# intelligent-machine-learning/dlrover

Measured on AMD Instinct MI355X. Metric: checkpoint save+restore sec and goodput % under injected failure, Llama-3-8B FSDP 1/2/4/8 MI355X, higher is better.
Workload: dtype bf16; 1 GPU; model=llama3_8b, params=8030261248, global_batch=2, seq_len=4096, parallelism=fsdp1, ckpt_interval=2, ckpt_scope=full, ckpt_restored_step=1

## Files before the change

dlrover_amd/ops/api.py:

```python

from typing import Optional, Tuple

import torch

_EXT = None
_EXT_ERR: Optional[str] = None


class ExtensionMissingError(RuntimeError):
    pass


def hip_ops():
    global _EXT, _EXT_ERR
    if _EXT is None and _EXT_ERR is None:
        try:
            from dlrover_amd.ops import _hip_ops as ext

            _EXT = ext
        except ImportError as e:
            _EXT_ERR = str(e)
    if _EXT is None:
        raise ExtensionMissingError(
            "dlrover_amd._hip_ops is not built — run "
# ... 208 lines not shown
    max_pos: int, head_dim: int, base: float = 500000.0, device="cpu"
) -> Tuple[torch.Tensor, torch.Tensor]:
    inv_freq = 1.0 / (
        base ** (torch.arange(0, head_dim, 2, dtype=torch.float32) / head_dim)
    )
    t = torch.arange(max_pos, dtype=torch.float32)
    freqs = torch.outer(t, inv_freq)
    return freqs.cos().to(device), freqs.sin().to(device)


class _CausalSoftmax(torch.autograd.Function):
    @staticmethod
    def forward(ctx, scores, scale, q_offset, q_len):
        q_len = q_len or scores.shape[-2]
        if _use_hip(scores):
            probs = scores.contiguous()
            hip_ops().causal_softmax_fwd(probs, q_len, q_offset, scale)
        else:
            probs = causal_softmax_ref(scores, scale, q_offset, q_len)
        ctx.save_for_backward(probs)
        ctx.scale = scale
        return probs

    @staticmethod
    def backward(ctx, dprobs):
        (probs,) = ctx.saved_tensors
        if _use_hip(probs):
            ds = dprobs.contiguous().clone()
            hip_ops().causal_softmax_bwd(ds, probs, ctx.scale)
            return ds, None, None, None
        pf, df = probs.float(), dprobs.float()
        dot = (pf * df).sum(-1, keepdim=True)
        return (pf * (df - dot) * ctx.scale).to(probs.dtype), None, None, None


def causal_softmax(
    scores: torch.Tensor, scale: float, q_offset: int = 0, q_len: int = 0
) -> torch.Tensor:
    return _CausalSoftmax.apply(scores, scale, q_offset, q_len)


def flash_attention_ref(
    q: torch.Tensor, k: torch.Tensor, v: torch.Tensor, scale: float
) -> torch.Tensor:
    B, H, S, D = q.shape
    rep = H // k.shape[1]
    kf = k.float().repeat_interleave(rep, 1)
    vf = v.float().repeat_interleave(rep, 1)
    s_ = torch.matmul(q.float(), kf.transpose(-1, -2)) * scale
    mask = torch.triu(torch.ones(S, S, dtype=torch.bool, device=q.device), 1)
    s_ = s_.masked_fill(mask, float("-inf"))
    p = torch.softmax(s_, -1)
    return torch.matmul(p, vf).to(q.dtype)


class _FlashAttention(torch.autograd.Function):
    @staticmethod
    def forward(ctx, q, k, v, scale):
        if _use_hip(q):
            if q.stride(-1) != 1:
                q = q.contiguous()
            if k.stride(-1) != 1:
                k = k.contiguous()
            if v.stride(-1) != 1:
                v = v.contiguous()
            out, lse = hip_ops().flash_attn_fwd(q, k, v, scale)
            ctx.save_for_backward(q, k, v, out, lse)
            ctx.scale = scale
            ctx.use_hip = True
            return out
        ctx.use_hip = False
        q32 = q.detach().clone().requires_grad_(True)
        k32 = k.detach().clone().requires_grad_(True)
        v32 = v.detach().clone().requires_grad_(True)
        with torch.enable_grad():
            out = flash_attention_ref(q32, k32, v32, scale)
        ctx.saved_ref = (q32, k32, v32, out)
        return out.detach()

    @staticmethod
    def backward(ctx, dout):
        if ctx.use_hip:
            q, k, v, out, lse = ctx.saved_tensors
            dq, dk, dv = hip_ops().flash_attn_bwd(
                q, k, v, out, dout.contiguous(), lse, ctx.scale
            )
            return dq, dk, dv, None
        q32, k32, v32, out = ctx.saved_ref
        torch.autograd.backward(out, dout)
        return q32.grad, k32.grad, v32.grad, None


def flash_attention(
    q: torch.Tensor, k: torch.Tensor, v: torch.Tensor, scale: float
) -> torch.Tensor:
    return _FlashAttention.apply(q, k, v, scale)


class _CrossEntropy(torch.autograd.Function):
    @staticmethod
    def forward(ctx, logits, targets, ignore_index):
        n_valid = int((targets != ignore_index).sum())
        grad_scale = 1.0 / max(n_valid, 1)
        if _use_hip(logits):
            work = logits.contiguous()
            losses = hip_ops().cross_entropy_fwd_bwd(
                work, targets.int(), ignore_index, grad_scale, True
            )
            ctx.save_for_backward(work)
            ctx.use_hip = True
        else:
            lf = logits.float()
            losses = torch.nn.functional.cross_entropy(
                lf.view(-1, lf.shape[-1]),
                targets.view(-1).long(),
                ignore_index=ignore_index,
                reduction="none",
            )
            dl = torch.softmax(lf, dim=-1)
            t = targets.view(-1)
            valid = t != ignore_index
            onehot = torch.zeros_like(dl.view(-1, dl.shape[-1]))
            onehot[valid, t[valid].long()] = 1.0
            dl = (dl.view(-1, dl.shape[-1]) - onehot) * grad_scale
            dl[~valid] = 0
            ctx.save_for_backward(dl.to(logits.dtype).view_as(logits))
            ctx.use_hip = False
        ctx.n_valid = n_valid
        return losses.sum() * grad_scale

    @staticmethod
    def backward(ctx, dloss):
        (dlogits,) = ctx.saved_tensors
        return dlogits * dloss, None, None


def cross_entropy_loss(
    logits: torch.Tensor, targets: torch.Tensor, ignore_index: int = -100
) -> torch.Tensor:
    return _CrossEntropy.apply(logits, targets, ignore_index)




def ce_shard_stats(
    logits_shard: torch.Tensor,
    targets: torch.Tensor,
    vocab_start: int,
    ignore_index: int = -100,
) -> torch.Tensor:
    vs = logits_shard.shape[-1]
    if _use_hip(logits_shard):
        return hip_ops().ce_shard_stats(
            logits_shard.view(-1, vs), targets.reshape(-1).int(), vocab_start,
            ignore_index,
        )
    x = logits_shard.detach().reshape(-1, vs).float()
    t = targets.reshape(-1).long()
    m = x.amax(-1)
    s = torch.exp(x - m[:, None]).sum(-1)
    local = t - vocab_start
    owns = (t != ignore_index) & (local >= 0) & (local < vs)
    picked = x.gather(1, torch.where(owns, local, 0)[:, None]).squeeze(1)
    return torch.stack([m, s, torch.where(owns, picked, 0.0)], dim=1)


def ce_shard_finish(
    logits_shard: torch.Tensor,
# ... 231 lines not shown
```

dlrover_amd/ops/csrc/attention_bwd_v3.hip:

```cpp
#include <cstdlib>
#include "kern_common.h"

typedef __attribute__((ext_vector_type(8))) __bf16 bf16x8;
typedef __attribute__((ext_vector_type(16))) float f32x16_t;
typedef __attribute__((ext_vector_type(2))) unsigned int u32x2_t;
typedef __attribute__((ext_vector_type(4))) unsigned int u32x4_t;
typedef __attribute__((ext_vector_type(2))) __bf16 bf16x2;

#define FB_D 128
#define FB_QB 256
#define FB_T 64

__device__ __forceinline__ int swzb(int row, int byte_col) {
  return byte_col ^ ((row & 7) << 4);
}

__device__ __forceinline__ unsigned pk_bf16(float lo, float hi) {
  bf16x2 v = {(__bf16)lo, (__bf16)hi};
  return *reinterpret_cast<unsigned*>(&v);
}

__device__ __forceinline__ bf16x8 trT_frag(const char* lds, int rb, int n,
                                           int lane, int half) {
  const int j = (lane & 15) >> 2;
  const int dq = n * 8 + ((lane & 16) >> 2) + (lane & 3);
  const int r0 = rb + half * 8 + j;
  const int r1 = r0 + 4;
  const unsigned base = (unsigned)(uintptr_t)lds;
  const unsigned a0 = base + r0 * 256 + ((dq * 8) ^ ((r0 & 7) << 4));
  const unsigned a1 = base + r1 * 256 + ((dq * 8) ^ ((r1 & 7) << 4));
  u32x2_t w0, w1;
  asm volatile(
      "ds_read_b64_tr_b16 %0, %2\n\t"
      "ds_read_b64_tr_b16 %1, %3\n\t"
      "s_waitcnt lgkmcnt(0)"
      : "=v"(w0), "=v"(w1)
      : "v"(a0), "v"(a1));
  u32x4_t frag = u32x4_t{w0.x, w0.y, w1.x, w1.y};
  return *reinterpret_cast<bf16x8*>(&frag);
}

__device__ __forceinline__ void pairswap_frags(const float v16[16], int half,
                                               bf16x8 out[2]) {
#pragma unroll
  for (int ks2 = 0; ks2 < 2; ++ks2) {
    const int r0 = ks2 * 8;
    unsigned w0 = pk_bf16(v16[r0 + 0], v16[r0 + 1]);
    unsigned w1 = pk_bf16(v16[r0 + 2], v16[r0 + 3]);
    unsigned w2 = pk_bf16(v16[r0 + 4], v16[r0 + 5]);
    unsigned w3 = pk_bf16(v16[r0 + 6], v16[r0 + 7]);
    u32x2_t s0 = __builtin_amdgcn_permlane32_swap(w0, w2, false, false);
    u32x2_t s1 = __builtin_amdgcn_permlane32_swap(w1, w3, false, false);
    u32x4_t frag = u32x4_t{s0.x, s1.x, s0.y, s1.y};
    out[ks2] = *reinterpret_cast<bf16x8*>(&frag);
  }
  (void)half;
}


__global__ __launch_bounds__(512) void fa_bwd_dq_v3_kernel(
    const short* __restrict__ q, const short* __restrict__ k,
    const short* __restrict__ v, const short* __restrict__ dout,
    const float* __restrict__ lse, const float* __restrict__ dvec,
    short* __restrict__ dq, int B, int H, int HKV, int S, float scale,
    long long qs_b, long long qs_h, long long qs_s,
    long long ks_b, long long ks_h, long long ks_s,
    long long vs_b, long long vs_h, long long vs_s,
    long long ds_b, long long ds_h, long long ds_s) {
  __shared__ char k_lds[2][FB_T * FB_D * 2];
  __shared__ char v_lds[2][FB_T * FB_D * 2];

  const int tid = threadIdx.x;
  const int wave = tid >> 6;
  const int lane = tid & 63;
  const int half = lane >> 5;
  const int qcol = lane & 31;

  const int qt = blockIdx.x;
  const int h = blockIdx.y;
  const int b = blockIdx.z;
  const int g = h / (H / HKV);

  const short* q_blk = q + (long long)b * qs_b + (long long)h * qs_h +
                       (long long)(qt * FB_QB) * qs_s;
  const short* do_blk = dout + (long long)b * ds_b + (long long)h * ds_h +
                        (long long)(qt * FB_QB) * ds_s;
  const short* k_head = k + (long long)b * ks_b + (long long)g * ks_h;
  const short* v_head = v + (long long)b * vs_b + (long long)g * vs_h;

  const int q_row_w = wave * 32 + qcol;
  const int q_glob = qt * FB_QB + q_row_w;

  bf16x8 bq[8], bdo[8];
#pragma unroll
  for (int ks = 0; ks < 8; ++ks) {
    bq[ks] = *reinterpret_cast<const bf16x8*>(
        q_blk + (long long)q_row_w * qs_s + ks * 16 + half * 8);
    bdo[ks] = *reinterpret_cast<const bf16x8*>(
        do_blk + (long long)q_row_w * ds_s + ks * 16 + half * 8);
  }
  const long long lrow = ((long long)b * H + h) * S + q_glob;
  const float L = lse[lrow];
  const float Dv = dvec[lrow];

  f32x16_t acc_dq[4];
#pragma unroll
  for (int n = 0; n < 4; ++n)
#pragma unroll
    for (int r = 0; r < 16; ++r) acc_dq[n][r] = 0.f;

  bf16x8 st_k[2], st_v[2];
  const int st_row0 = (tid * 16) / FB_D;
  const int st_col0 = (tid * 16) % FB_D;
  auto issue_loads = [&](int kt) {
    const short* ksrc = k_head + (long long)(kt * FB_T) * ks_s;
    const short* vsrc = v_head + (long long)(kt * FB_T) * vs_s;
#pragma unroll
    for (int c = 0; c < 2; ++c) {
      st_k[c] = *reinterpret_cast<const bf16x8*>(
          ksrc + (long long)st_row0 * ks_s + st_col0 + c * 8);
      st_v[c] = *reinterpret_cast<const bf16x8*>(
          vsrc + (long long)st_row0 * vs_s + st_col0 + c * 8);
    }
  };
  auto write_lds = [&](int buf) {
#pragma unroll
    for (int c = 0; c < 2; ++c) {
      const int col = st_col0 + c * 8;
      *reinterpret_cast<bf16x8*>(k_lds[buf] + st_row0 * 256 +
                                 swzb(st_row0, col * 2)) = st_k[c];
      *reinterpret_cast<bf16x8*>(v_lds[buf] + st_row0 * 256 +
                                 swzb(st_row0, col * 2)) = st_v[c];
    }
  };

  const int n_tiles = (qt + 1) * (FB_QB / FB_T);
  const int wave_q_max = qt * FB_QB + wave * 32 + 31;

  issue_loads(0);
  write_lds(0);
  __syncthreads();

  for (int kt = 0; kt < n_tiles; ++kt) {
    const int cur = kt & 1;
    const char* k_cur = k_lds[cur];
    const char* v_cur = v_lds[cur];
    if (kt + 1 < n_tiles) issue_loads(kt + 1);

    const int kv0 = kt * FB_T;
    if (kv0 <= wave_q_max) {
      bf16x8 bds[4];
#pragma unroll
      for (int n = 0; n < 2; ++n) {
        f32x16_t acc_s;
#pragma unroll
        for (int r = 0; r < 16; ++r) acc_s[r] = 0.f;
#pragma unroll
        for (int ks = 0; ks < 8; ++ks) {
          const int row = n * 32 + qcol;
          bf16x8 ak = *reinterpret_cast<const bf16x8*>(
              k_cur + row * 256 + swzb(row, (ks * 16 + half * 8) * 2));
          acc_s = __builtin_amdgcn_mfma_f32_32x32x16_bf16(ak, bq[ks], acc_s,
                                                          0, 0, 0);
        }
#pragma unroll
        for (int r = 0; r < 16; ++r) {
          const int kv_glob = kv0 + n * 32 + (r & 3) + 8 * (r >> 2) + 4 * half;
          acc_s[r] =
              (kv_glob > q_glob) ? 0.f : __expf(acc_s[r] * scale - L);
        }
        f32x16_t acc_dp;
#pragma unroll
        for (int r = 0; r < 16; ++r) acc_dp[r] = 0.f;
#pragma unroll
        for (int ks = 0; ks < 8; ++ks) {
          const int row = n * 32 + qcol;
          bf16x8 av = *reinterpret_cast<const bf16x8*>(
              v_cur + row * 256 + swzb(row, (ks * 16 + half * 8) * 2));
          acc_dp = __builtin_amdgcn_mfma_f32_32x32x16_bf16(av, bdo[ks],
                                                           acc_dp, 0, 0, 0);
        }
        float dsv[16];
#pragma unroll
        for (int r = 0; r < 16; ++r)
          dsv[r] = acc_s[r] * (acc_dp[r] - Dv) * scale;
        pairswap_frags(dsv, half, &bds[n * 2]);
      }
#pragma unroll
      for (int n = 0; n < 4; ++n) {
#pragma unroll
        for (int ks = 0; ks < 4; ++ks) {
          bf16x8 akT = trT_frag(k_cur, ks * 16, n, lane, half);
          acc_dq[n] = __builtin_amdgcn_mfma_f32_32x32x16_bf16(
              akT, bds[ks], acc_dq[n], 0, 0, 0);
        }
      }
    }

    __syncthreads();
    if (kt + 1 < n_tiles) {
      write_lds(cur ^ 1);
      __syncthreads();
    }
  }

  short* dq_blk = dq + (long long)b * qs_b + (long long)h * qs_h +
                  (long long)(qt * FB_QB) * qs_s;
  char* slab = (char*)k_lds + (wave & 3) * (32 * FB_D * 2);
  for (int round = 0; round < 2; ++round) {
    __syncthreads();
    if ((wave >> 2) == round) {
#pragma unroll
      for (int n = 0; n < 4; ++n) {
#pragma unroll
        for (int r = 0; r < 16; ++r) {
          const int d = n * 32 + (r & 3) + 8 * (r >> 2) + 4 * half;
          *reinterpret_cast<__bf16*>(slab + qcol * 256 + swzb(qcol, d * 2)) =
              (__bf16)acc_dq[n][r];
        }
      }
    }
    __syncthreads();
    if ((wave >> 2) == round) {
#pragma unroll
      for (int pass = 0; pass < 4; ++pass) {
        const int elem0 = (pass * 64 + lane) * 16;
        const int r2 = elem0 / FB_D;
        const int c2 = elem0 % FB_D;
        bf16x8 v0 = *reinterpret_cast<const bf16x8*>(
            slab + r2 * 256 + swzb(r2, c2 * 2));
        bf16x8 v1 = *reinterpret_cast<const bf16x8*>(
            slab + r2 * 256 + swzb(r2, (c2 + 8) * 2));
        short* dst = dq_blk + (long long)(wave * 32 + r2) * qs_s + c2;
        *reinterpret_cast<bf16x8*>(dst) = v0;
        *reinterpret_cast<bf16x8*>(dst + 8) = v1;
      }
    }
  }
}


#define FB_DKV_PROLOGUE()                                                    \
  __shared__ char q_lds[FB_T * FB_D * 2];                                    \
  __shared__ char do_lds[FB_T * FB_D * 2];                                   \
  __shared__ float l_lds[FB_T];                                              \
  __shared__ float d_lds[FB_T];                                              \
  const int tid = threadIdx.x;                                               \
  const int wave = tid >> 6;                                                 \
  const int lane = tid & 63;                                                 \
  const int half = lane >> 5;                                                \
  const int kcol = lane & 31;                                                \
  const int kvb0 = blockIdx.x * FB_QB;                                       \
  const int chunk = blockIdx.y;                                              \
  const int CH = gridDim.y;                                                  \
  const int bg = blockIdx.z;                                                 \
  const int b = bg / HKV;                                                    \
  const int g = bg % HKV;                                                    \
  const int rep = H / HKV;                                                   \
  const int kv_own = kvb0 + wave * 32 + kcol;                                \
  const short* k_head = k + (long long)b * ks_b + (long long)g * ks_h;       \
  bf16x8 bk[8];                                                              \
  _Pragma("unroll") for (int ks = 0; ks < 8; ++ks) bk[ks] =                  \
      *reinterpret_cast<const bf16x8*>(k_head + (long long)kv_own * ks_s +   \
                                       ks * 16 + half * 8);                  \
  const int qt_min = kvb0 / FB_T;                                            \
  const int n_qt = S / FB_T - qt_min;                                        \
  const int n_work = rep * n_qt;                                             \
  const int wave_kv_min = kvb0 + wave * 32;                                  \
  auto stage_qdo = [&](int h, int qt) {                                      \
    const short* qsrc = q + (long long)b * qs_b + (long long)h * qs_h +      \
                        (long long)(qt * FB_T) * qs_s;                       \
    const short* dsrc = dout + (long long)b * ds_b + (long long)h * ds_h +   \
                        (long long)(qt * FB_T) * ds_s;                       \
    _Pragma("unroll") for (int c = 0; c < 2; ++c) {                          \
      const int linear = (tid * 16) + c * 8;                                 \
      const int row = linear / FB_D;                                         \
      const int col = linear % FB_D;                                         \
      *reinterpret_cast<bf16x8*>(q_lds + row * 256 + swzb(row, col * 2)) =   \
          *reinterpret_cast<const bf16x8*>(qsrc + (long long)row * qs_s +    \
                                           col);                             \
      *reinterpret_cast<bf16x8*>(do_lds + row * 256 + swzb(row, col * 2)) =  \
          *reinterpret_cast<const bf16x8*>(dsrc + (long long)row * ds_s +    \
                                           col);                             \
    }                                                                        \
    if (tid < FB_T) {                                                        \
      const long long lrow = ((long long)b * H + h) * S + qt * FB_T + tid;   \
      l_lds[tid] = lse[lrow];                                                \
      d_lds[tid] = dvec[lrow];                                               \
    }                                                                        \
  }

__global__ __launch_bounds__(512) void fa_bwd_dv_v3_kernel(
    const short* __restrict__ q, const short* __restrict__ k,
    const short* __restrict__ v, const short* __restrict__ dout,
    const float* __restrict__ lse, const float* __restrict__ dvec,
    float* __restrict__ dk32, float* __restrict__ dv32, int B, int H,
    int HKV, int S, float scale,
    long long qs_b, long long qs_h, long long qs_s,
    long long ks_b, long long ks_h, long long ks_s,
    long long vs_b, long long vs_h, long long vs_s,
    long long ds_b, long long ds_h, long long ds_s) {
  FB_DKV_PROLOGUE();

  {
    f32x16_t acc_dv[4];
#pragma unroll
    for (int n = 0; n < 4; ++n)
#pragma unroll
      for (int r = 0; r < 16; ++r) acc_dv[n][r] = 0.f;

    for (int w = chunk; w < n_work; w += CH) {
      const int h = g * rep + w / n_qt;
      const int qt = qt_min + w % n_qt;
      __syncthreads();
      stage_qdo(h, qt);
      __syncthreads();
      if (qt * FB_T + FB_T - 1 < wave_kv_min) continue;
#pragma unroll
      for (int st = 0; st < 2; ++st) {
        const int q0 = qt * FB_T + st * 32;
        if (q0 + 31 < wave_kv_min) continue;
        f32x16_t acc_s;
#pragma unroll
        for (int r = 0; r < 16; ++r) acc_s[r] = 0.f;
#pragma unroll
        for (int ks = 0; ks < 8; ++ks) {
          const int row = st * 32 + kcol;
          bf16x8 aq = *reinterpret_cast<const bf16x8*>(
              q_lds + (st * 32 + kcol) * 256 +
              swzb(st * 32 + kcol, (ks * 16 + half * 8) * 2));
          (void)row;
          acc_s = __builtin_amdgcn_mfma_f32_32x32x16_bf16(aq, bk[ks], acc_s,
                                                          0, 0, 0);
        }
        float pv[16];
#pragma unroll
        for (int r = 0; r < 16; ++r) {
          const int qrow = st * 32 + (r & 3) + 8 * (r >> 2) + 4 * half;
          const int q_glob = qt * FB_T + qrow;
          pv[r] = (kv_own > q_glob)
                      ? 0.f
                      : __expf(acc_s[r] * scale - l_lds[qrow]);
        }
        bf16x8 bp[2];
        pairswap_frags(pv, half, bp);
#pragma unroll
        for (int n = 0; n < 4; ++n) {
#pragma unroll
          for (int ks2 = 0; ks2 < 2; ++ks2) {
            bf16x8 adoT =
                trT_frag(do_lds, st * 32 + ks2 * 16, n, lane, half);
            acc_dv[n] = __builtin_amdgcn_mfma_f32_32x32x16_bf16(
                adoT, bp[ks2], acc_dv[n], 0, 0, 0);
          }
        }
      }
    }
    float* dv_base = dv32 + ((long long)bg * S + kv_own) * FB_D;
#pragma unroll
    for (int n = 0; n < 4; ++n)
#pragma unroll
      for (int r = 0; r < 16; ++r) {
        const int d = n * 32 + (r & 3) + 8 * (r >> 2) + 4 * half;
        atomicAdd(dv_base + d, acc_dv[n][r]);
      }
  }

}

__global__ __launch_bounds__(512) void fa_bwd_dk_v3_kernel(
    const short* __restrict__ q, const short* __restrict__ k,
    const short* __restrict__ v, const short* __restrict__ dout,
    const float* __restrict__ lse, const float* __restrict__ dvec,
    float* __restrict__ dk32, float* __restrict__ dv32, int B, int H,
    int HKV, int S, float scale,
    long long qs_b, long long qs_h, long long qs_s,
    long long ks_b, long long ks_h, long long ks_s,
    long long vs_b, long long vs_h, long long vs_s,
    long long ds_b, long long ds_h, long long ds_s) {
  FB_DKV_PROLOGUE();
  const short* v_head = v + (long long)b * vs_b + (long long)g * vs_h;
  bf16x8 bv[8];
#pragma unroll
  for (int ks = 0; ks < 8; ++ks)
    bv[ks] = *reinterpret_cast<const bf16x8*>(
        v_head + (long long)kv_own * vs_s + ks * 16 + half * 8);

  {
    f32x16_t acc_dk[4];
#pragma unroll
    for (int n = 0; n < 4; ++n)
#pragma unroll
      for (int r = 0; r < 16; ++r) acc_dk[n][r] = 0.f;

    for (int w = chunk; w < n_work; w += CH) {
      const int h = g * rep + w / n_qt;
      const int qt = qt_min + w % n_qt;
      __syncthreads();
      stage_qdo(h, qt);
      __syncthreads();
      if (qt * FB_T + FB_T - 1 < wave_kv_min) continue;
#pragma unroll
      for (int st = 0; st < 2; ++st) {
        const int q0 = qt * FB_T + st * 32;
        if (q0 + 31 < wave_kv_min) continue;
        f32x16_t acc_s, acc_dp;
#pragma unroll
        for (int r = 0; r < 16; ++r) acc_s[r] = acc_dp[r] = 0.f;
#pragma unroll
        for (int ks = 0; ks < 8; ++ks) {
          const int row = st * 32 + kcol;
          const int bc = (ks * 16 + half * 8) * 2;
          bf16x8 aq = *reinterpret_cast<const bf16x8*>(
              q_lds + row * 256 + swzb(row, bc));
          acc_s = __builtin_amdgcn_mfma_f32_32x32x16_bf16(aq, bk[ks], acc_s,
                                                          0, 0, 0);
          bf16x8 ado = *reinterpret_cast<const bf16x8*>(
              do_lds + row * 256 + swzb(row, bc));
          acc_dp = __builtin_amdgcn_mfma_f32_32x32x16_bf16(ado, bv[ks],
                                                           acc_dp, 0, 0, 0);
        }
        float dsv[16];
#pragma unroll
        for (int r = 0; r < 16; ++r) {
          const int qrow = st * 32 + (r & 3) + 8 * (r >> 2) + 4 * half;
          const int q_glob = qt * FB_T + qrow;
          const float p = (kv_own > q_glob)
                              ? 0.f
                              : __expf(acc_s[r] * scale - l_lds[qrow]);
          dsv[r] = p * (acc_dp[r] - d_lds[qrow]) * scale;
        }
        bf16x8 bds[2];
        pairswap_frags(dsv, half, bds);
#pragma unroll
        for (int n = 0; n < 4; ++n) {
#pragma unroll
          for (int ks2 = 0; ks2 < 2; ++ks2) {
            bf16x8 aqT = trT_frag(q_lds, st * 32 + ks2 * 16, n, lane, half);
            acc_dk[n] = __builtin_amdgcn_mfma_f32_32x32x16_bf16(
                aqT, bds[ks2], acc_dk[n], 0, 0, 0);
          }
        }
      }
    }
    float* dk_base = dk32 + ((long long)bg * S + kv_own) * FB_D;
#pragma unroll
    for (int n = 0; n < 4; ++n)
#pragma unroll
      for (int r = 0; r < 16; ++r) {
        const int d = n * 32 + (r & 3) + 8 * (r >> 2) + 4 * half;
        atomicAdd(dk_base + d, acc_dk[n][r]);
      }
  }
}

extern "C" void fa_bwd_dkv_v3_launch(const void* q, const void* k,
                                     const void* v, const void* dout,
                                     const void* lse, const void* dvec,
                                     void* dk32, void* dv32, int B, int H,
                                     int HKV, int S, float scale,
                                     const long long* strides,
                                     hipStream_t stream) {
  const int kv_blocks = S / FB_QB;
  int ch = 1;
  while (kv_blocks * ch * B * HKV < 512 && ch < 16) ch <<= 1;
  dim3 grid(kv_blocks, ch, B * HKV);
  hipLaunchKernelGGL(fa_bwd_dv_v3_kernel, grid, dim3(512), 0, stream,
                     (const short*)q, (const short*)k, (const short*)v,
                     (const short*)dout, (const float*)lse,
                     (const float*)dvec, (float*)dk32, (float*)dv32, B, H,
                     HKV, S, scale, strides[0], strides[1], strides[2],
                     strides[3], strides[4], strides[5], strides[6],
                     strides[7], strides[8], strides[9], strides[10],
                     strides[11]);
  hipLaunchKernelGGL(fa_bwd_dk_v3_kernel, grid, dim3(512), 0, stream,
                     (const short*)q, (const short*)k, (const short*)v,
                     (const short*)dout, (const float*)lse,
                     (const float*)dvec, (float*)dk32, (float*)dv32, B, H,
                     HKV, S, scale, strides[0], strides[1], strides[2],
                     strides[3], strides[4], strides[5], strides[6],
                     strides[7], strides[8], strides[9], strides[10],
                     strides[11]);
}

extern "C" void fa_bwd_dq_v3_launch(const void* q, const void* k,
                                    const void* v, const void* dout,
                                    const void* lse, const void* dvec,
                                    void* dq, int B, int H, int HKV, int S,
                                    float scale, const long long* strides,
                                    hipStream_t stream) {
  dim3 grid(S / FB_QB, H, B);
  hipLaunchKernelGGL(fa_bwd_dq_v3_kernel, grid, dim3(512), 0, stream,
                     (const short*)q, (const short*)k, (const short*)v,
                     (const short*)dout, (const float*)lse,
                     (const float*)dvec, (short*)dq, B, H, HKV, S, scale,
                     strides[0], strides[1], strides[2], strides[3],
                     strides[4], strides[5], strides[6], strides[7],
                     strides[8], strides[9], strides[10], strides[11]);
}
```

dlrover_amd/ops/csrc/attention_v3.hip:

```cpp
#include <cstdlib>
#include "kern_common.h"

typedef __attribute__((ext_vector_type(8))) __bf16 bf16x8;
typedef __attribute__((ext_vector_type(4))) float f32x4_t;
typedef __attribute__((ext_vector_type(16))) float f32x16_t;
typedef __attribute__((ext_vector_type(2))) unsigned int u32x2_t;
typedef __attribute__((ext_vector_type(4))) unsigned int u32x4_t;
typedef __attribute__((ext_vector_type(2))) __bf16 bf16x2;

#define FA3_D 128
#define FA3_QB 256
#define FA3_QW 32
#define FA3_KT 64

__device__ __forceinline__ int swz3(int row, int byte_col) {
  return byte_col ^ ((row & 7) << 4);
}

__device__ __forceinline__ unsigned pack_bf16(float lo, float hi) {
  bf16x2 v = {(__bf16)lo, (__bf16)hi};
  return *reinterpret_cast<unsigned*>(&v);
}

__device__ __forceinline__ bf16x8 tr_colT_frag(const char* lds, int rb,
                                               int n, int lane, int half) {
  typedef __attribute__((ext_vector_type(2))) unsigned int u32x2_;
  const int j = (lane & 15) >> 2;
  const int dq = n * 8 + ((lane & 16) >> 2) + (lane & 3);
  const int r0 = rb + half * 8 + j;
  const int r1 = r0 + 4;
  const unsigned base = (unsigned)(uintptr_t)lds;
  const unsigned a0 = base + r0 * 256 + ((dq * 8) ^ ((r0 & 7) << 4));
  const unsigned a1 = base + r1 * 256 + ((dq * 8) ^ ((r1 & 7) << 4));
  u32x2_ w0, w1;
  asm volatile(
      "ds_read_b64_tr_b16 %0, %2\n\t"
      "ds_read_b64_tr_b16 %1, %3\n\t"
      "s_waitcnt lgkmcnt(0)"
      : "=v"(w0), "=v"(w1)
      : "v"(a0), "v"(a1));
  u32x4_t frag = u32x4_t{w0.x, w0.y, w1.x, w1.y};
  return *reinterpret_cast<bf16x8*>(&frag);
}

template <bool TRV>
__global__ __launch_bounds__(512) void flash_attn_fwd_v3_kernel(
    const short* __restrict__ q, const short* __restrict__ k,
    const short* __restrict__ v, short* __restrict__ out,
    float* __restrict__ lse, int B, int H, int HKV, int S, float scale,
    long long qs_b, long long qs_h, long long qs_s,
    long long ks_b, long long ks_h, long long ks_s,
    long long vs_b, long long vs_h, long long vs_s,
    long long os_b, long long os_h, long long os_s) {
  __shared__ char k_lds[2][FA3_KT * FA3_D * 2];
  __shared__ char vt_lds[2][FA3_D * FA3_KT * 2];

  const int tid = threadIdx.x;
  const int wave = tid >> 6;
  const int lane = tid & 63;
  const int half = lane >> 5;
  const int qcol = lane & 31;

  const int qt = blockIdx.x;
  const int h = blockIdx.y;
  const int b = blockIdx.z;
  const int g = h / (H / HKV);

  const short* q_blk = q + (long long)b * qs_b + (long long)h * qs_h +
                       (long long)(qt * FA3_QB) * qs_s;
  const short* k_head = k + (long long)b * ks_b + (long long)g * ks_h;
  const short* v_head = v + (long long)b * vs_b + (long long)g * vs_h;

  const int q_row_w = wave * FA3_QW + qcol;
  bf16x8 bq[8];
#pragma unroll
  for (int ks = 0; ks < 8; ++ks) {
    const short* src =
        q_blk + (long long)q_row_w * qs_s + ks * 16 + half * 8;
    bq[ks] = *reinterpret_cast<const bf16x8*>(src);
  }

  const int q_glob = qt * FA3_QB + q_row_w;
  float m_run = -1e30f, l_run = 0.f;
  f32x16_t acc_o[4];
#pragma unroll
  for (int n = 0; n < 4; ++n)
#pragma unroll
    for (int r = 0; r < 16; ++r) acc_o[n][r] = 0.f;

  bf16x8 st_k[2], st_v[2];
  const int st_row0 = (tid * 16) / FA3_D;
  const int st_col0 = (tid * 16) % FA3_D;

  auto issue_loads = [&](int kt) {
    const short* ksrc = k_head + (long long)(kt * FA3_KT) * ks_s;
    const short* vsrc = v_head + (long long)(kt * FA3_KT) * vs_s;
#pragma unroll
    for (int c = 0; c < 2; ++c) {
      st_k[c] = *reinterpret_cast<const bf16x8*>(
          ksrc + (long long)st_row0 * ks_s + st_col0 + c * 8);
      st_v[c] = *reinterpret_cast<const bf16x8*>(
          vsrc + (long long)st_row0 * vs_s + st_col0 + c * 8);
    }
  };

  auto write_lds = [&](int buf) {
    char* kb = k_lds[buf];
    char* vb = vt_lds[buf];
#pragma unroll
    for (int c = 0; c < 2; ++c) {
      const int col = st_col0 + c * 8;
      *reinterpret_cast<bf16x8*>(kb + st_row0 * 256 + swz3(st_row0, col * 2)) =
          st_k[c];
      if (TRV) {
        *reinterpret_cast<bf16x8*>(vb + st_row0 * 256 +
                                   swz3(st_row0, col * 2)) = st_v[c];
      } else {
#pragma unroll
        for (int i = 0; i < 8; ++i) {
          const int trow = col + i;
          *reinterpret_cast<__bf16*>(vb + trow * 128 +
                                     swz3(trow, st_row0 * 2)) = st_v[c][i];
        }
      }
    }
  };

  const int n_tiles = (qt + 1) * (FA3_QB / FA3_KT);
  const int wave_q_max = qt * FA3_QB + wave * FA3_QW + FA3_QW - 1;

  issue_loads(0);
  write_lds(0);
  __syncthreads();

  for (int kt = 0; kt < n_tiles; ++kt) {
    const int cur = kt & 1;
    const char* k_cur = k_lds[cur];
    const char* vt_cur = vt_lds[cur];
    if (kt + 1 < n_tiles) issue_loads(kt + 1);

    const int kv0 = kt * FA3_KT;
    const bool wave_active = kv0 <= wave_q_max;

    if (wave_active) {
      f32x16_t acc_s[2];
#pragma unroll
      for (int n = 0; n < 2; ++n)
#pragma unroll
        for (int r = 0; r < 16; ++r) acc_s[n][r] = 0.f;
// ... 69 lines not shown
          const int r0 = n * 16 + ks2 * 8;
          unsigned w0 = pack_bf16(p[r0 + 0], p[r0 + 1]);
          unsigned w1 = pack_bf16(p[r0 + 2], p[r0 + 3]);
          unsigned w2 = pack_bf16(p[r0 + 4], p[r0 + 5]);
          unsigned w3 = pack_bf16(p[r0 + 6], p[r0 + 7]);
          u32x2_t s0 = __builtin_amdgcn_permlane32_swap(w0, w2, false, false);
          u32x2_t s1 = __builtin_amdgcn_permlane32_swap(w1, w3, false, false);
          u32x4_t frag = u32x4_t{s0.x, s1.x, s0.y, s1.y};
          bp[n * 2 + ks2] = *reinterpret_cast<bf16x8*>(&frag);
        }
      }

#pragma unroll
      for (int n = 0; n < 4; ++n) {
#pragma unroll
        for (int ks = 0; ks < 4; ++ks) {
          bf16x8 av;
          if (TRV) {
            av = tr_colT_frag(vt_cur, ks * 16, n, lane, half);
          } else {
            const int row = n * 32 + qcol;
            const int byte_col = (ks * 16 + half * 8) * 2;
            av = *reinterpret_cast<const bf16x8*>(
                vt_cur + row * 128 + swz3(row, byte_col));
          }
          acc_o[n] = __builtin_amdgcn_mfma_f32_32x32x16_bf16(av, bp[ks],
                                                             acc_o[n], 0, 0, 0);
        }
      }
    }

    __syncthreads();
    if (kt + 1 < n_tiles) {
      write_lds(cur ^ 1);
      __syncthreads();
    }
  }

  const float inv = l_run > 0.f ? 1.f / l_run : 0.f;
  short* o_blk = out + (long long)b * os_b + (long long)h * os_h +
                 (long long)(qt * FA3_QB) * os_s;
  char* slab = (char*)k_lds + (wave & 3) * (FA3_QW * FA3_D * 2);
  for (int round = 0; round < 2; ++round) {
    __syncthreads();
    if ((wave >> 2) == round) {
#pragma unroll
      for (int n = 0; n < 4; ++n) {
#pragma unroll
        for (int r = 0; r < 16; ++r) {
          const int d = n * 32 + (r & 3) + 8 * (r >> 2) + 4 * half;
          *reinterpret_cast<__bf16*>(slab + qcol * 256 + swz3(qcol, d * 2)) =
              (__bf16)(acc_o[n][r] * inv);
        }
      }
    }
    __syncthreads();
    if ((wave >> 2) == round) {
#pragma unroll
      for (int pass = 0; pass < 4; ++pass) {
        const int elem0 = (pass * 64 + lane) * 16;
        const int r2 = elem0 / FA3_D;
        const int c2 = elem0 % FA3_D;
        bf16x8 v0 = *reinterpret_cast<const bf16x8*>(
            slab + r2 * 256 + swz3(r2, c2 * 2));
        bf16x8 v1 = *reinterpret_cast<const bf16x8*>(
            slab + r2 * 256 + swz3(r2, (c2 + 8) * 2));
        short* dst = o_blk + (long long)(wave * FA3_QW + r2) * os_s + c2;
        *reinterpret_cast<bf16x8*>(dst) = v0;
        *reinterpret_cast<bf16x8*>(dst + 8) = v1;
      }
    }
  }
  if (half == 0 && lse != nullptr) {
    const long long lrow = ((long long)b * H + h) * S + q_glob;
    lse[lrow] = m_run + __logf(fmaxf(l_run, 1e-30f));
  }
}

extern "C" void flash_attn_fwd_v3_launch(const void* q, const void* k,
                                         const void* v, void* out, void* lse,
                                         int B, int H, int HKV, int S,
                                         float scale, const long long* strides,
                                         hipStream_t stream) {
  dim3 grid(S / FA3_QB, H, B);
  static const bool trv = []() {
    const char* e = getenv("DLROVER_FA_TRV");
    return e == nullptr || e[0] != '0';
  }();
  if (trv) {
    hipLaunchKernelGGL((flash_attn_fwd_v3_kernel<true>), grid, dim3(512), 0,
                       stream, (const short*)q, (const short*)k,
                       (const short*)v, (short*)out, (float*)lse, B, H, HKV,
                       S, scale, strides[0], strides[1], strides[2],
                       strides[3], strides[4], strides[5], strides[6],
                       strides[7], strides[8], strides[9], strides[10],
                       strides[11]);
  } else {
    hipLaunchKernelGGL((flash_attn_fwd_v3_kernel<false>), grid, dim3(512), 0,
                       stream, (const short*)q, (const short*)k,
                       (const short*)v, (short*)out, (float*)lse, B, H, HKV,
                       S, scale, strides[0], strides[1], strides[2],
                       strides[3], strides[4], strides[5], strides[6],
                       strides[7], strides[8], strides[9], strides[10],
                       strides[11]);
  }
}
```

dlrover_amd/ops/csrc/bindings.cpp:

```cpp
#include <torch/extension.h>
#include <ATen/cuda/CUDAContext.h>

#include <tuple>
#include <vector>

extern "C" {
void rmsnorm_fwd_launch(const void*, const void*, void*, void*, int, int,
                        float, void*);
void rmsnorm_add_fwd_launch(const void*, const void*, const void*, void*,
                            void*, void*, int, int, float, void*);
void rmsnorm_bwd_launch(const void*, const void*, const void*, const void*,
                        const void*, void*, void*, void*, void*, int, int,
                        int, void*);
void rope_launch(void*, const void*, const void*, const void*, long long,
                 long long, int, int, int, void*);
void rope_oop_launch(const void*, void*, const void*, const void*,
                     const void*, long long, long long, int, int, long long,
                     int, void*);
void swiglu_fwd_launch(const void*, void*, long long, int, void*);
void swiglu_bwd_launch(const void*, const void*, void*, long long, int, void*);
void adamw_launch(void*, const void*, void*, void*, void*, long long, float,
                  float, float, float, float, int, int, float, void*);
void causal_softmax_fwd_launch(void*, long long, int, int, int, float, void*);
void causal_softmax_bwd_launch(void*, const void*, long long, int, float,
// ... 221 lines not shown
  TORCH_CHECK(row_len % 8 == 0, "row_len must be a multiple of 8");
  const long long n_rows = scores.numel() / row_len;
  causal_softmax_fwd_launch(scores.data_ptr(), n_rows, row_len, (int)q_len,
                            (int)q_offset, (float)scale, cur_stream());
}

void causal_softmax_bwd(at::Tensor& dscores, const at::Tensor& probs,
                        double scale) {
  check_bf16(dscores, "dscores");
  check_bf16(probs, "probs");
  const int row_len = (int)dscores.size(-1);
  const long long n_rows = dscores.numel() / row_len;
  causal_softmax_bwd_launch(dscores.data_ptr(), probs.data_ptr(), n_rows,
                            row_len, (float)scale, cur_stream());
}

static void check_attn_view(const at::Tensor& t, const char* name) {
  TORCH_CHECK(t.is_cuda() && t.scalar_type() == at::kBFloat16, name,
              " must be bf16 GPU");
  TORCH_CHECK(t.dim() == 4 && t.stride(3) == 1, name,
              " must be [B,H,S,D] with contiguous D");
}

static void pack_strides(long long* st, const at::Tensor& t, int at) {
  st[at + 0] = (long long)t.stride(0);
  st[at + 1] = (long long)t.stride(1);
  st[at + 2] = (long long)t.stride(2);
}

std::tuple<at::Tensor, at::Tensor> flash_attn_fwd(const at::Tensor& q,
                                                  const at::Tensor& k,
                                                  const at::Tensor& v,
                                                  double scale) {
  check_attn_view(q, "q");
  check_attn_view(k, "k");
  check_attn_view(v, "v");
  const int B = (int)q.size(0), H = (int)q.size(1), S = (int)q.size(2);
  const int D = (int)q.size(3), HKV = (int)k.size(1);
  TORCH_CHECK(D == 128, "flash_attn: head_dim must be 128");
  TORCH_CHECK(S % 64 == 0, "flash_attn: seq len must be a multiple of 64");
  TORCH_CHECK(H % HKV == 0, "flash_attn: H % HKV != 0");
  auto out_bshd = at::empty({B, S, H, D}, q.options());
  auto out = out_bshd.permute({0, 2, 1, 3});
  auto lse = at::empty({B, H, S}, q.options().dtype(at::kFloat));
  long long st[12];
  pack_strides(st, q, 0);
  pack_strides(st, k, 3);
  pack_strides(st, v, 6);
  pack_strides(st, out, 9);
  static const bool use_v2 = []() {
    const char* e = getenv("DLROVER_FA_V2");
    return e != nullptr && e[0] == '1';
  }();
  static const bool v3_enabled = []() {
    const char* e = getenv("DLROVER_FA_V3");
    return e == nullptr || e[0] != '0';
  }();
  if (v3_enabled && !use_v2 && S % 256 == 0) {
    flash_attn_fwd_v3_launch(q.data_ptr(), k.data_ptr(), v.data_ptr(),
                             out_bshd.data_ptr(), lse.data_ptr(), B, H, HKV,
                             S, (float)scale, st, cur_stream());
  } else if (use_v2) {
    flash_attn_fwd_v2_launch(q.data_ptr(), k.data_ptr(), v.data_ptr(),
                             out_bshd.data_ptr(), lse.data_ptr(), B, H, HKV,
                             S, (float)scale, st, cur_stream());
  } else {
    flash_attn_fwd_launch(q.data_ptr(), k.data_ptr(), v.data_ptr(),
                          out_bshd.data_ptr(), lse.data_ptr(), B, H, HKV, S,
                          (float)scale, st, cur_stream());
  }
  return {out, lse};
}

std::tuple<at::Tensor, at::Tensor, at::Tensor> flash_attn_bwd(
    const at::Tensor& q, const at::Tensor& k, const at::Tensor& v,
    const at::Tensor& out, const at::Tensor& dout_in, const at::Tensor& lse,
    double scale) {
  check_attn_view(q, "q");
  check_attn_view(k, "k");
  check_attn_view(v, "v");
  const int B = (int)q.size(0), H = (int)q.size(1), S = (int)q.size(2);
  const int D = (int)q.size(3), HKV = (int)k.size(1);
  at::Tensor dout = dout_in;
  if (dout.strides() != out.strides()) {
    dout = at::empty_like(out.permute({0, 2, 1, 3}).contiguous())
               .view({B, S, H, D});
    dout = dout.permute({0, 2, 1, 3});
    dout.copy_(dout_in);
  }
  TORCH_CHECK(dout.stride(3) == 1, "dout needs contiguous D");
  auto dvec = at::empty({B, H, S}, q.options().dtype(at::kFloat));
  {
    long long ost[3], dstr[3];
    pack_strides(ost, out, 0);
    pack_strides(dstr, dout, 0);
    fa_bwd_pre_launch(dout.data_ptr(), out.data_ptr(), dvec.data_ptr(), B, H,
                      S, ost, dstr, cur_stream());
    long long st[12];
    pack_strides(st, q, 0);
    pack_strides(st, k, 3);
    pack_strides(st, v, 6);
    pack_strides(st, dout, 9);
    auto dq_bshd = at::empty({B, S, H, D}, q.options());
    auto dq = dq_bshd.permute({0, 2, 1, 3});
    {
      long long stq[12];
      pack_strides(stq, dq, 0);
      pack_strides(stq, k, 3);
      pack_strides(stq, v, 6);
      pack_strides(stq, dout, 9);
      at::Tensor quse = q;
      if (q.strides() != dq.strides()) {
        auto q_bshd = at::empty({B, S, H, D}, q.options());
        auto qv = q_bshd.permute({0, 2, 1, 3});
        qv.copy_(q);
        quse = qv;
        pack_strides(stq, quse, 0);
      }
      static const bool bwd_v3 = []() {
        const char* e = getenv("DLROVER_FA_BWD_V3");
        return e == nullptr || e[0] != '0';
      }();
      auto dk32 = at::zeros({B, HKV, S, D}, k.options().dtype(at::kFloat));
      auto dv32 = at::zeros({B, HKV, S, D}, v.options().dtype(at::kFloat));
      if (bwd_v3 && S % 256 == 0) {
        fa_bwd_dq_v3_launch(quse.data_ptr(), k.data_ptr(), v.data_ptr(),
                            dout.data_ptr(), lse.data_ptr(), dvec.data_ptr(),
                            dq_bshd.data_ptr(), B, H, HKV, S, (float)scale,
                            stq, cur_stream());
        fa_bwd_dkv_v3_launch(quse.data_ptr(), k.data_ptr(), v.data_ptr(),
                             dout.data_ptr(), lse.data_ptr(),
                             dvec.data_ptr(), dk32.data_ptr(),
                             dv32.data_ptr(), B, H, HKV, S, (float)scale,
                             stq, cur_stream());
      } else {
        fa_bwd_dq_launch(quse.data_ptr(), k.data_ptr(), v.data_ptr(),
                         dout.data_ptr(), lse.data_ptr(), dvec.data_ptr(),
                         dq_bshd.data_ptr(), B, H, HKV, S, (float)scale, stq,
                         cur_stream());
        fa_bwd_dkv_launch(quse.data_ptr(), k.data_ptr(), v.data_ptr(),
                          dout.data_ptr(), lse.data_ptr(), dvec.data_ptr(),
                          dk32.data_ptr(), dv32.data_ptr(), B, H, HKV, S,
                          (float)scale, stq, cur_stream());
      }
      auto dk = at::empty({B, HKV, S, D}, k.options());
      auto dv = at::empty({B, HKV, S, D}, v.options());
      f32_to_bf16_launch(dk32.data_ptr(), dk.data_ptr(), dk32.numel(),
                         cur_stream());
      f32_to_bf16_launch(dv32.data_ptr(), dv.data_ptr(), dv32.numel(),
                         cur_stream());
      return {dq, dk, dv};
    }
  }
}

at::Tensor mfma16_probe(const at::Tensor& A, const at::Tensor& B) {
  check_bf16(A, "A");
  check_bf16(B, "B");
  TORCH_CHECK(A.sizes() == at::IntArrayRef({16, 32}) &&
              B.sizes() == at::IntArrayRef({32, 16}),
              "probe wants A[16,32], B[32,16]");
  auto C = at::empty({16, 16}, A.options().dtype(at::kFloat));
  mfma16_probe_launch(A.data_ptr(), B.data_ptr(), C.data_ptr(), cur_stream());
  return C;
}

void memcpy_d2h_async(int64_t dst_addr, const at::Tensor& src) {
// ... 294 lines not shown
```

dlrover_amd/ops/csrc/kern_common.h:

```cpp
#pragma once

#include <hip/hip_runtime.h>
#include <hip/hip_bf16.h>

#define WAVE_SIZE 64

typedef __attribute__((ext_vector_type(2))) short short2_t;
typedef __attribute__((ext_vector_type(4))) short short4_t;
typedef __attribute__((ext_vector_type(8))) short short8_t;
typedef __attribute__((ext_vector_type(4))) float float4_t;

using bf16_t = __hip_bfloat16;

__device__ __forceinline__ float bf2f(short bits) {
  union { unsigned int u; float f; } cvt;
  cvt.u = ((unsigned int)(unsigned short)bits) << 16;
  return cvt.f;
}

__device__ __forceinline__ short f2bf(float f) {
  union { unsigned int u; float f; } cvt;
  cvt.f = f;
  unsigned int u = cvt.u;
  unsigned int rounding = 0x7FFFu + ((u >> 16) & 1u);
  u += rounding;
  return (short)(u >> 16);
}

__device__ __forceinline__ void load8(const short* p, float out[8]) {
  short8_t v = *reinterpret_cast<const short8_t*>(p);
#pragma unroll
  for (int j = 0; j < 8; ++j) out[j] = bf2f(v[j]);
}

__device__ __forceinline__ void store8(short* p, const float in[8]) {
  short8_t v;
#pragma unroll
  for (int j = 0; j < 8; ++j) v[j] = f2bf(in[j]);
  *reinterpret_cast<short8_t*>(p) = v;
}


__device__ __forceinline__ float wave_reduce_sum(float v) {
#pragma unroll
  for (int off = 32; off > 0; off >>= 1) v += __shfl_xor(v, off, WAVE_SIZE);
  return v;
}

__device__ __forceinline__ float wave_reduce_max(float v) {
#pragma unroll
  for (int off = 32; off > 0; off >>= 1) v = fmaxf(v, __shfl_xor(v, off, WAVE_SIZE));
  return v;
}

__device__ __forceinline__ float block_reduce_sum(float v, float* scratch) {
  const int lane = threadIdx.x & (WAVE_SIZE - 1);
  const int wid = threadIdx.x >> 6;
  const int nwaves = (blockDim.x + WAVE_SIZE - 1) >> 6;
  v = wave_reduce_sum(v);
  if (lane == 0) scratch[wid] = v;
  __syncthreads();
  float total = 0.f;
#pragma unroll 4
  for (int i = 0; i < nwaves; ++i) total += scratch[i];
  __syncthreads();
  return total;
}

__device__ __forceinline__ float block_reduce_max(float v, float* scratch) {
  const int lane = threadIdx.x & (WAVE_SIZE - 1);
  const int wid = threadIdx.x >> 6;
  const int nwaves = (blockDim.x + WAVE_SIZE - 1) >> 6;
  v = wave_reduce_max(v);
  if (lane == 0) scratch[wid] = v;
  __syncthreads();
  float m = -INFINITY;
#pragma unroll 4
  for (int i = 0; i < nwaves; ++i) m = fmaxf(m, scratch[i]);
  __syncthreads();
  return m;
}

__host__ __forceinline__ int grid_capped(long long work_items, int block) {
  long long blocks = (work_items + block - 1) / block;
  if (blocks > 2048) blocks = 2048;
  if (blocks < 1) blocks = 1;
  return (int)blocks;
}

#define HIP_CHECK_KERNEL()                                                 \
  do {                                                                     \
    hipError_t e = hipGetLastError();                                      \
    if (e != hipSuccess) {                                                 \
      printf("dlrover_amd kernel launch failed: %s\n", hipGetErrorString(e)); \
    }                                                                      \
  } while (0)
```

Measured before the change: 59.94 goodput_percent.

## Rework flash-attention kernels: builtin LDS transpose reads, reversed 1D grids, vectorized LSE loads

Swaps inline-asm ds_read_b64_tr_b16, which carried an unconditional waitcnt, for the compiler builtin so the scheduler can overlap the reads. Flattens the forward, dq and dkv grids to 1D, with query tiles issued in reverse (longest causal tiles first) and heads grouped by KV head for cache reuse. Vectorizes LSE/D loads from LDS in the dkv kernels and skips the dout copy when its strides are already usable. The workload metric is checkpoint goodput, so attention-kernel changes affect it only through step time.

```diff
diff --git a/dlrover_amd/ops/api.py b/dlrover_amd/ops/api.py
--- a/dlrover_amd/ops/api.py
+++ b/dlrover_amd/ops/api.py
@@ -314,8 +314,10 @@
     def backward(ctx, dout):
         if ctx.use_hip:
             q, k, v, out, lse = ctx.saved_tensors
+            if dout.stride(-1) != 1:
+                dout = dout.contiguous()
             dq, dk, dv = hip_ops().flash_attn_bwd(
-                q, k, v, out, dout.contiguous(), lse, ctx.scale
+                q, k, v, out, dout, lse, ctx.scale
             )
             return dq, dk, dv, None
         q32, k32, v32, out = ctx.saved_ref
diff --git a/dlrover_amd/ops/csrc/attention_bwd_v3.hip b/dlrover_amd/ops/csrc/attention_bwd_v3.hip
--- a/dlrover_amd/ops/csrc/attention_bwd_v3.hip
+++ b/dlrover_amd/ops/csrc/attention_bwd_v3.hip
@@ -29,15 +29,10 @@
   const unsigned base = (unsigned)(uintptr_t)lds;
   const unsigned a0 = base + r0 * 256 + ((dq * 8) ^ ((r0 & 7) << 4));
   const unsigned a1 = base + r1 * 256 + ((dq * 8) ^ ((r1 & 7) << 4));
-  u32x2_t w0, w1;
-  asm volatile(
-      "ds_read_b64_tr_b16 %0, %2\n\t"
-      "ds_read_b64_tr_b16 %1, %3\n\t"
-      "s_waitcnt lgkmcnt(0)"
-      : "=v"(w0), "=v"(w1)
-      : "v"(a0), "v"(a1));
-  u32x4_t frag = u32x4_t{w0.x, w0.y, w1.x, w1.y};
-  return *reinterpret_cast<bf16x8*>(&frag);
+  const short4_t w0 = lds_read_tr16_b64(a0);
+  const short4_t w1 = lds_read_tr16_b64(a1);
+  return __builtin_bit_cast(
+      bf16x8, __builtin_shufflevector(w0, w1, 0, 1, 2, 3, 4, 5, 6, 7));
 }
 
 __device__ __forceinline__ void pairswap_frags(const float v16[16], int half,
@@ -76,10 +71,15 @@
   const int half = lane >> 5;
   const int qcol = lane & 31;
 
-  const int qt = blockIdx.x;
-  const int h = blockIdx.y;
-  const int b = blockIdx.z;
-  const int g = h / (H / HKV);
+  const int nq = S / FB_QB;
+  const int bh = B * H;
+  const int bg_n = B * HKV;
+  const int qt = nq - 1 - (int)blockIdx.x / bh;
+  const int jj = (int)blockIdx.x % bh;
+  const int gi = jj % bg_n;
+  const int b = gi / HKV;
+  const int g = gi % HKV;
+  const int h = g * (H / HKV) + jj / bg_n;
 
   const short* q_blk = q + (long long)b * qs_b + (long long)h * qs_h +
                        (long long)(qt * FB_QB) * qs_s;
@@ -243,17 +243,20 @@
 #define FB_DKV_PROLOGUE()                                                    \
   __shared__ char q_lds[FB_T * FB_D * 2];                                    \
   __shared__ char do_lds[FB_T * FB_D * 2];                                   \
-  __shared__ float l_lds[FB_T];                                              \
-  __shared__ float d_lds[FB_T];                                              \
+  __shared__ __attribute__((aligned(16))) float l_lds[FB_T];                 \
+  __shared__ __attribute__((aligned(16))) float d_lds[FB_T];                 \
   const int tid = threadIdx.x;                                               \
   const int wave = tid >> 6;                                                 \
   const int lane = tid & 63;                                                 \
   const int half = lane >> 5;                                                \
   const int kcol = lane & 31;                                                \
-  const int kvb0 = blockIdx.x * FB_QB;                                       \
-  const int chunk = blockIdx.y;                                              \
-  const int CH = gridDim.y;                                                  \
-  const int bg = blockIdx.z;                                                 \
+   \
+   \
+   \
+  const int per_kvb = CH * B * HKV;                                          \
+  const int kvb0 = ((int)blockIdx.x / per_kvb) * FB_QB;                      \
+  const int chunk = ((int)blockIdx.x % per_kvb) / (B * HKV);                 \
+  const int bg = ((int)blockIdx.x % per_kvb) % (B * HKV);                    \
   const int b = bg / HKV;                                                    \
   const int g = bg % HKV;                                                    \
   const int rep = H / HKV;                                                   \
@@ -295,7 +298,7 @@
     const short* __restrict__ v, const short* __restrict__ dout,
     const float* __restrict__ lse, const float* __restrict__ dvec,
     float* __restrict__ dk32, float* __restrict__ dv32, int B, int H,
-    int HKV, int S, float scale,
+    int HKV, int S, int CH, float scale,
     long long qs_b, long long qs_h, long long qs_s,
     long long ks_b, long long ks_h, long long ks_s,
     long long vs_b, long long vs_h, long long vs_s,
@@ -333,14 +336,17 @@
           acc_s = __builtin_amdgcn_mfma_f32_32x32x16_bf16(aq, bk[ks], acc_s,
                                                           0, 0, 0);
         }
+        float lrow[16];
+#pragma unroll
+        for (int r = 0; r < 16; ++r)
+          lrow[r] = l_lds[st * 32 + (r & 3) + 8 * (r >> 2) + 4 * half];
         float pv[16];
 #pragma unroll
         for (int r = 0; r < 16; ++r) {
           const int qrow = st * 32 + (r & 3) + 8 * (r >> 2) + 4 * half;
           const int q_glob = qt * FB_T + qrow;
-          pv[r] = (kv_own > q_glob)
-                      ? 0.f
-                      : __expf(acc_s[r] * scale - l_lds[qrow]);
+          const float e = __expf(acc_s[r] * scale - lrow[r]);
+          pv[r] = (kv_own > q_glob) ? 0.f : e;
         }
         bf16x8 bp[2];
         pairswap_frags(pv, half, bp);
@@ -373,7 +379,7 @@
     const short* __restrict__ v, const short* __restrict__ dout,
     const float* __restrict__ lse, const float* __restrict__ dvec,
     float* __restrict__ dk32, float* __restrict__ dv32, int B, int H,
-    int HKV, int S, float scale,
+    int HKV, int S, int CH, float scale,
     long long qs_b, long long qs_h, long long qs_s,
     long long ks_b, long long ks_h, long long ks_s,
     long long vs_b, long long vs_h, long long vs_s,
@@ -422,13 +428,19 @@
         }
         float dsv[16];
 #pragma unroll
-        for (int r = 0; r < 16; ++r) {
-          const int qrow = st * 32 + (r & 3) + 8 * (r >> 2) + 4 * half;
-          const int q_glob = qt * FB_T + qrow;
-          const float p = (kv_own > q_glob)
-                              ? 0.f
-                              : __expf(acc_s[r] * scale - l_lds[qrow]);
-          dsv[r] = p * (acc_dp[r] - d_lds[qrow]) * scale;
+        for (int j = 0; j < 4; ++j) {
+          const int qrow0 = st * 32 + 8 * j + 4 * half;
+          const float4_t l4 = *reinterpret_cast<const float4_t*>(l_lds + qrow0);
+          const float4_t d4 = *reinterpret_cast<const float4_t*>(d_lds + qrow0);
+#pragma unroll
+          for (int i = 0; i < 4; ++i) {
+            const int r = j * 4 + i;
+            const int q_glob = qt * FB_T + qrow0 + i;
+            const float e = __expf(acc_s[r] * scale - l4[i]);
+            const float p = (kv_own > q_glob) ? 0.f : e;
+            dsv[r] = p * (acc_dp[r] - d4[i]) * scale;
+          }
+          __builtin_amdgcn_sched_barrier(0);
         }
         bf16x8 bds[2];
         pairswap_frags(dsv, half, bds);
@@ -464,12 +476,12 @@
   const int kv_blocks = S / FB_QB;
   int ch = 1;
   while (kv_blocks * ch * B * HKV < 512 && ch < 16) ch <<= 1;
-  dim3 grid(kv_blocks, ch, B * HKV);
+  dim3 grid(kv_blocks * ch * B * HKV);
   hipLaunchKernelGGL(fa_bwd_dv_v3_kernel, grid, dim3(512), 0, stream,
                      (const short*)q, (const short*)k, (const short*)v,
                      (const short*)dout, (const float*)lse,
                      (const float*)dvec, (float*)dk32, (float*)dv32, B, H,
-                     HKV, S, scale, strides[0], strides[1], strides[2],
+                     HKV, S, ch, scale, strides[0], strides[1], strides[2],
                      strides[3], strides[4], strides[5], strides[6],
                      strides[7], strides[8], strides[9], strides[10],
                      strides[11]);
@@ -477,7 +489,7 @@
                      (const short*)q, (const short*)k, (const short*)v,
                      (const short*)dout, (const float*)lse,
                      (const float*)dvec, (float*)dk32, (float*)dv32, B, H,
-                     HKV, S, scale, strides[0], strides[1], strides[2],
+                     HKV, S, ch, scale, strides[0], strides[1], strides[2],
                      strides[3], strides[4], strides[5], strides[6],
                      strides[7], strides[8], strides[9], strides[10],
                      strides[11]);
@@ -489,7 +501,7 @@
                                     void* dq, int B, int H, int HKV, int S,
                                     float scale, const long long* strides,
                                     hipStream_t stream) {
-  dim3 grid(S / FB_QB, H, B);
+  dim3 grid((S / FB_QB) * H * B);
   hipLaunchKernelGGL(fa_bwd_dq_v3_kernel, grid, dim3(512), 0, stream,
                      (const short*)q, (const short*)k, (const short*)v,
                      (const short*)dout, (const float*)lse,
diff --git a/dlrover_amd/ops/csrc/attention_v3.hip b/dlrover_amd/ops/csrc/attention_v3.hip
--- a/dlrover_amd/ops/csrc/attention_v3.hip
+++ b/dlrover_amd/ops/csrc/attention_v3.hip
@@ -24,7 +24,6 @@
 
 __device__ __forceinline__ bf16x8 tr_colT_frag(const char* lds, int rb,
                                                int n, int lane, int half) {
-  typedef __attribute__((ext_vector_type(2))) unsigned int u32x2_;
   const int j = (lane & 15) >> 2;
   const int dq = n * 8 + ((lane & 16) >> 2) + (lane & 3);
   const int r0 = rb + half * 8 + j;
@@ -32,15 +31,10 @@
   const unsigned base = (unsigned)(uintptr_t)lds;
   const unsigned a0 = base + r0 * 256 + ((dq * 8) ^ ((r0 & 7) << 4));
   const unsigned a1 = base + r1 * 256 + ((dq * 8) ^ ((r1 & 7) << 4));
-  u32x2_ w0, w1;
-  asm volatile(
-      "ds_read_b64_tr_b16 %0, %2\n\t"
-      "ds_read_b64_tr_b16 %1, %3\n\t"
-      "s_waitcnt lgkmcnt(0)"
-      : "=v"(w0), "=v"(w1)
-      : "v"(a0), "v"(a1));
-  u32x4_t frag = u32x4_t{w0.x, w0.y, w1.x, w1.y};
-  return *reinterpret_cast<bf16x8*>(&frag);
+  const short4_t w0 = lds_read_tr16_b64(a0);
+  const short4_t w1 = lds_read_tr16_b64(a1);
+  return __builtin_bit_cast(
+      bf16x8, __builtin_shufflevector(w0, w1, 0, 1, 2, 3, 4, 5, 6, 7));
 }
 
 template <bool TRV>
@@ -61,10 +55,15 @@
   const int half = lane >> 5;
   const int qcol = lane & 31;
 
-  const int qt = blockIdx.x;
-  const int h = blockIdx.y;
-  const int b = blockIdx.z;
-  const int g = h / (H / HKV);
+  const int nq = S / FA3_QB;
+  const int bh = B * H;
+  const int bg_n = B * HKV;
+  const int qt = nq - 1 - (int)blockIdx.x / bh;
+  const int jj = (int)blockIdx.x % bh;
+  const int gi = jj % bg_n;
+  const int b = gi / HKV;
+  const int g = gi % HKV;
+  const int h = g * (H / HKV) + jj / bg_n;
 
   const short* q_blk = q + (long long)b * qs_b + (long long)h * qs_h +
                        (long long)(qt * FA3_QB) * qs_s;
@@ -300,7 +299,7 @@
                                          int B, int H, int HKV, int S,
                                          float scale, const long long* strides,
                                          hipStream_t stream) {
-  dim3 grid(S / FA3_QB, H, B);
+  dim3 grid((S / FA3_QB) * H * B);
   static const bool trv = []() {
     const char* e = getenv("DLROVER_FA_TRV");
     return e == nullptr || e[0] != '0';
diff --git a/dlrover_amd/ops/csrc/bindings.cpp b/dlrover_amd/ops/csrc/bindings.cpp
--- a/dlrover_amd/ops/csrc/bindings.cpp
+++ b/dlrover_amd/ops/csrc/bindings.cpp
@@ -327,7 +327,11 @@
   const int B = (int)q.size(0), H = (int)q.size(1), S = (int)q.size(2);
   const int D = (int)q.size(3), HKV = (int)k.size(1);
   at::Tensor dout = dout_in;
-  if (dout.strides() != out.strides()) {
+  const bool dout_direct =
+      dout.stride(3) == 1 && dout.stride(0) % 8 == 0 &&
+      dout.stride(1) % 8 == 0 && dout.stride(2) % 8 == 0 &&
+      reinterpret_cast<uintptr_t>(dout.data_ptr()) % 16 == 0;
+  if (!dout_direct) {
     dout = at::empty_like(out.permute({0, 2, 1, 3}).contiguous())
                .view({B, S, H, D});
     dout = dout.permute({0, 2, 1, 3});
diff --git a/dlrover_amd/ops/csrc/kern_common.h b/dlrover_amd/ops/csrc/kern_common.h
--- a/dlrover_amd/ops/csrc/kern_common.h
+++ b/dlrover_amd/ops/csrc/kern_common.h
@@ -38,6 +38,12 @@
 #pragma unroll
   for (int j = 0; j < 8; ++j) v[j] = f2bf(in[j]);
   *reinterpret_cast<short8_t*>(p) = v;
+}
+
+__device__ __forceinline__ short4_t lds_read_tr16_b64(unsigned addr) {
+  typedef __attribute__((address_space(3))) short4_t lds_short4_t;
+  return __builtin_amdgcn_ds_read_tr16_b64_v4i16(
+      reinterpret_cast<lds_short4_t*>((uintptr_t)addr));
 }
 
 
```

After: 56.09 goodput_percent. -6.4%, worse.
